# andrewcharlesjones/spatial-alignment

Hardware: AMD Instinct MI355X
Metric: training steps/sec (ELBO fwd+bwd), 2-view N=10k M=200, 1/2/4/8 GPU (higher is better)
Workload: dtype f32 (fp64 warp layer, covariance whitening and M x M factorisations)

## Files before the change

### include/gpsa_hip.h

```cpp
#ifndef GPSA_HIP_H
#define GPSA_HIP_H

#ifdef __cplusplus
extern "C" {
#endif

enum {
  GPSA_F32 = 0,
  GPSA_F64 = 1,
  GPSA_F32_X64 = 2,
  GPSA_F32_OUT64 = 3,
  GPSA_F32_ACC64 = 4
};
enum { GPSA_K_RBF = 0, GPSA_K_MATERN12 = 1, GPSA_K_MATERN32 = 2 };
enum { GPSA_EINVAL = -1, GPSA_EWORKSPACE = -2, GPSA_EUNSUPPORTED = -3 };

int gpsa_version(void);
const char* gpsa_build_arch(void);
const char* gpsa_source_hash(void);

int gpsa_kmat(int dtype, int in_dtype, int kind, const void* Z, int M, const void* X, long long C,
              int D, const void* ls_u, const void* var_u, double jitter, void* K, void* stream);

long long gpsa_kmat_bwd_workspace(int dtype, int M, long long C, int D);
// ... 119 lines not shown
                    double* out, void* workspace, long long workspace_bytes, void* stream);
int gpsa_loglik_bwd(const float* F, const float* Y, const float* noise_u, const double* gout, int S,
                    long long N, int P, float* dF, float* dnoise_u, void* workspace,
                    long long workspace_bytes, void* stream);

int gpsa_bdot(int dtype, const void* A, long long strideA, const void* B, long long strideB,
              long long n, int batch, void* out, void* workspace, long long workspace_bytes,
              void* stream);
int gpsa_add_diag(int dtype, void* A, int M, int batch, double s, void* stream);

int gpsa_mvn_kl_fwd(const double* Kinv, const double* logdetK, const double* Omega,
                    long long omega_stride, const double* logdetO, long long logdet_stride,
                    const double* Dm, const double* KD, int M, int L, double* kl, void* stream);
int gpsa_mvn_kl_bwd(const double* Kuu, const double* Kinv, const double* Omega, long long omega_stride,
                    const double* Oinv, long long oinv_stride, const double* Dm, const double* KD,
                    const double* g, int M, int L, double* dOmega, double* dDm, double* Sp,
                    void* stream);

int gpsa_mvn_kl_grouped_fwd(const double* mats, const double* inv, const double* logdet,
                            const int* om_idx, const int* pr_idx, const double* D, int M, int T,
                            double* kl, double* KD, void* stream);
int gpsa_mvn_kl_grouped_bwd(const double* mats, const double* inv, const int* om_idx,
                            const int* pr_list, const int* grp_off, const int* order, const double* D,
                            const double* KD, const double* g, int M, int T, int P, double* dOmega,
                            double* dD, double* S, void* stream);

int gpsa_elbo_fwd(const double* ll, int n_ll, const double* kl, int n_kl, double kl_scale, float* loss,
                  void* stream);
int gpsa_elbo_bwd(const float* gloss, int n_ll, int n_kl, double kl_scale, double* dll, double* dkl,
                  void* stream);

long long gpsa_kmeans_workspace(long long N, int D, int K);
int gpsa_kmeans_assign(const float* X, long long N, int D, const float* centres, int K, int* assign,
                       float* d2, void* stream);
int gpsa_kmeans_update(const float* X, const int* assign, long long N, int D, int K, float* centres,
                       int* counts, void* workspace, long long workspace_bytes, void* stream);


int gpsa_kmat_batched(int kind, const float* Z, long long strideZ, int M, const float* X, long long strideX,
                      long long C, int D, const float* ls_u, const float* var_u, int stride_par,
                      const long long* n_live, int batch, double jitter, double* K, long long strideK,
                      void* stream);
long long gpsa_kmat_bwd_batched_workspace(int M, long long C, int D, int batch);
int gpsa_kmat_bwd_batched(int kind, const float* Z, long long strideZ, int M, const float* X, long long strideX,
                          long long C, int D, const float* ls_u, const float* var_u, int stride_par,
                          const long long* n_live, int batch, const double* Kbar, long long strideK, int same,
                          double* dZ, long long stride_dZ, double* dparams, void* workspace,
                          long long workspace_bytes, void* stream);
int gpsa_kmat_bwd_x64(int kind, const float* Z, int M, const double* X, long long C, int D, const float* ls_u,
                      const float* var_u, const float* Kbar, double* dZ, double* dX, double* dparams,
                      void* workspace, long long workspace_bytes, void* stream);
int gpsa_kmat_bwd_x64_f64(int kind, const float* Z, int M, const double* X, long long C, int D, const float* ls_u,
                          const float* var_u, const double* Kbar, double* dZ, double* dX, double* dparams,
                          void* workspace, long long workspace_bytes, void* stream);
int gpsa_kmat_bwd_x64_f64_axpy(int kind, const float* Z, int M, const double* X, long long C, int D, const float* ls_u,
                               const float* var_u, const double* Kbar, const double* X2, const float* d, double s,
                               double* dZ, double* dX, double* dparams, void* workspace, long long workspace_bytes,
                               void* stream);
long long gpsa_exact_dkuu_workspace(int M, long long C);
int gpsa_exact_dkuu_f64(const double* G, const double* A, const float* d, int M, long long C, double* dK,
                        void* workspace, long long workspace_bytes, void* stream);
long long gpsa_longk_f64_workspace(int M, long long K, int nprob);
int gpsa_longk_f64(int nprob, const double* const* G, const double* const* B, const void* const* d, int d_dtype,
                   int M, long long K, long long ld, int sym, const double* alpha, const double* beta,
                   double* const* out, void* workspace, long long workspace_bytes, void* stream);
int gpsa_kmat_bwd_x64_axpy(int kind, const float* Z, int M, const double* X, long long C, int D, const float* ls_u,
                           const float* var_u, const float* Kbar, const float* X2, const float* d, double s,
                           double* dZ, double* dX, double* dparams, void* workspace, long long workspace_bytes,
                           void* stream);
int gpsa_whiten_f64_dual(const double* Kinv, const double* Kuf, int M, long long C, double* alpha64, float* alpha32,
                         double* q, void* workspace, long long workspace_bytes, void* stream);

int gpsa_whiten_gen_f64_dual(const double* Kinv, int kind, const float* Z, const double* X64, int D, const float* ls_u,
                             const float* var_u, int M, long long C, double* alpha64, float* alpha32, double* q,
                             void* workspace, long long workspace_bytes, void* stream);
int gpsa_whiten_axpy_f32(const double* Kinv, const float* X, int M, long long C, const float* X2, const float* d,
                         double s, float* out, void* workspace, long long workspace_bytes, void* stream);
int gpsa_whiten_batched_f64(const double* Kinv, long long strideKinv, const double* Kuf, int M, long long C,
                            long long strideX, double* alpha, double* q, int batch, void* workspace,
                            long long workspace_bytes, void* stream);
int gpsa_quadform_fwd_keep_batched_f64(const double* alpha, const double* Omega, int M, long long C, int L,
                                       double* v, double* W, const double* dcT, double* meanT, int batch,
                                       void* stream);
int gpsa_quadform_bwd_alpha_kept_batched_f64(const double* W, const double* g, int M, long long C, int L,
                                             const double* dcT, const double* dmeanT, double* dalpha,
                                             int batch, void* stream);
int gpsa_col_axpy_batched_f64(const double* Y, const double* X, const double* d, double s, int M, long long C,
                              double* out, int batch, void* stream);
long long gpsa_gram_batched_workspace(int M, long long C, int L, int batch);
int gpsa_gram_batched_f64(const double* alpha, const double* g, int M, long long C, int L, double* dOmega,
                          int batch, void* workspace, long long workspace_bytes, void* stream);
int gpsa_mvn_kl_grouped_bwd_acc(const double* mats, const double* inv, const int* om_idx,
                                const int* pr_list, const int* grp_off, const int* order, const double* D,
                                const double* KD, const double* g, int M, int T, int P, double* dOmega,
                                double* dD, double* S, int accumulate, void* stream);

#define GPSA_MAX_MODS 4

typedef struct gpsa_step_desc {
  int n_views, n_dims, n_mods, n_samples;
  int m_x, m_g;
  int kind_warp, kind_data;
  int n_latent[GPSA_MAX_MODS];
  int n_out[GPSA_MAX_MODS];
  int has_lmc[GPSA_MAX_MODS];
  long long n_rows[GPSA_MAX_MODS];
  int s_test;
  long long n_test[GPSA_MAX_MODS];
  int want_kl;
  const int* view_fixed;
  const long long* view_rows;
  long long keep_budget_bytes;
  int exact_inducing_grad;
  int kl_own_lo, kl_own_hi;
  int contraction;
} gpsa_step_desc;

typedef struct gpsa_step_params {
  const float* Xtilde;
  const float* delta_G;
  const float* Omega_sqt_G;
  const float* warp_ls;
  const float* warp_var;
  const float* slopes;
  const float* intercepts;
  const float* Gtilde;
  const float* data_ls;
  const float* data_var;
  const float* Omega_sqt_F[GPSA_MAX_MODS];
  const float* delta_F[GPSA_MAX_MODS];
  const float* W[GPSA_MAX_MODS];
} gpsa_step_params;

typedef struct gpsa_step_param_grads {
  float *Xtilde, *delta_G, *Omega_sqt_G, *warp_ls, *warp_var, *Gtilde, *data_ls, *data_var;
  float* Omega_sqt_F[GPSA_MAX_MODS];
  float* delta_F[GPSA_MAX_MODS];
  float* W[GPSA_MAX_MODS];
} gpsa_step_param_grads;

typedef struct gpsa_step_io {
  const float* X[GPSA_MAX_MODS];
  const float* eps_G;
  const float* eps_F[GPSA_MAX_MODS];
  const float* G_test[GPSA_MAX_MODS];
  const float* eps_F_test[GPSA_MAX_MODS];
  float* G_means[GPSA_MAX_MODS];
  float* G_samples[GPSA_MAX_MODS];
  float* F_latent[GPSA_MAX_MODS];
  float* F_obs[GPSA_MAX_MODS];
  float* F_latent_test[GPSA_MAX_MODS];
  float* F_obs_test[GPSA_MAX_MODS];
  float* mu_z;
  double* kl;
  int* flag;
  int keep_products;
  int reuse_mm;
  int fuse_elbo;
  const float* Y[GPSA_MAX_MODS];
  const float* noise_u[GPSA_MAX_MODS];
  double* ll_part[GPSA_MAX_MODS];
  float* F_fused_T[GPSA_MAX_MODS];
  double* bwd_acc;
  int bwd_acc_mode;
  void* f_event;
  const float* loss_src;
// ... 88 lines not shown
```

### spatial_alignment_amd/_lib.py

```python
import ctypes as C
import os

_HERE = os.path.dirname(os.path.abspath(__file__))
LIB_PATH = os.path.join(_HERE, "libgpsa_hip.so")

_vp, _i, _ll, _d = C.c_void_p, C.c_int, C.c_longlong, C.c_double

SIGNATURES = {
    "gpsa_version": (_i, []),
    "gpsa_build_arch": (C.c_char_p, []),
    "gpsa_source_hash": (C.c_char_p, []),
    "gpsa_kmat": (_i, [_i, _i, _i, _vp, _i, _vp, _ll, _i, _vp, _vp, _d, _vp, _vp]),
    "gpsa_kmat_bwd_workspace": (_ll, [_i, _i, _ll, _i]),
    "gpsa_kmat_bwd": (_i, [_i, _i, _i, _vp, _i, _vp, _ll, _i, _vp, _vp, _vp, _i, _vp, _vp, _vp, _vp, _ll, _vp]),
    "gpsa_gemm_workspace": (_ll, [_i, _i, _i, _i, _i]),
    "gpsa_gemm": (_i, [_i, _i, _i, _i, _i, _ll, _d, _vp, _ll, _ll, _vp, _ll, _ll, _d, _vp, _ll, _ll,
                       _i, _i, _vp, _ll, _vp]),
    "gpsa_omega_fwd": (_i, [_vp, _i, _i, _d, _vp, _vp]),
    "gpsa_omega_bwd": (_i, [_vp, _vp, _i, _i, _i, _vp, _vp]),
    "gpsa_omega_fwd2": (_i, [_vp, _i, _vp, _vp, _i, _vp, _i, _d, _vp]),
    "gpsa_omega_bwd2": (_i, [_vp, _vp, _vp, _i, _vp, _vp, _vp, _i, _i, _i, _vp]),
    "gpsa_chol_f64": (_i, [_vp, _i, _i, _vp, _vp, _vp]),
    "gpsa_tri_inv_f64": (_i, [_vp, _vp, _i, _i, _vp]),
    "gpsa_chol_inv_f64": (_i, [_vp, _vp, _i, _i, _vp, _vp, _vp]),
    "gpsa_experiment_split_bf16_product": (_i, [_vp, _vp, _i, _ll, _i, _i, _vp, _vp]),
    "gpsa_experiment_split_bf16_rate": (_i, [_i, _i, _vp, _vp]),
    "gpsa_chol_inv_sel_f64": (_i, [_vp, _vp, _i, _i, _i, _i, _i, _vp, _vp, _vp]),
    "gpsa_chol_inv_blocked_workspace": (_ll, [_i, _i]),
    "gpsa_chol_inv_blocked_f64": (_i, [_vp, _vp, _i, _i, _vp, _vp, _vp, _ll, _vp]),
    "gpsa_quadform_workspace": (_ll, [_i, _i, _ll, _i]),
    "gpsa_quadform_fwd": (_i, [_i, _i, _vp, _vp, _i, _ll, _i, _vp, _vp, _ll, _vp]),
    "gpsa_quadform_bwd_alpha": (_i, [_i, _i, _vp, _vp, _vp, _i, _ll, _i, _vp, _vp, _ll, _vp]),
    "gpsa_quadform_fwd_keep": (_i, [_i, _vp, _vp, _i, _ll, _i, _vp, _vp, _vp, _vp, _vp]),
    "gpsa_quadform_bwd_alpha_kept": (_i, [_i, _vp, _vp, _i, _ll, _i, _vp, _vp, _vp, _vp]),
    "gpsa_quadform_bwd_omega": (_i, [_i, _i, _vp, _vp, _i, _ll, _i, _vp, _vp, _ll, _vp]),
    "gpsa_quadform_bwd_omega_takes_delta": (_i, [_i, _ll]),
    "gpsa_quadform_bwd_omega_delta_f32": (_i, [_i, _vp, _vp, _vp, _i, _ll, _i, _vp, _vp, _d, _vp, _ll, _vp]),
    "gpsa_quadform_bwd_omega_x3_workspace": (_ll, [_i, _ll, _i]),
    "gpsa_quadform_bwd_omega_x3": (_i, [_i, _i, _vp, _vp, _i, _ll, _i, _vp, _vp, _ll, _vp]),
    "gpsa_quadform_bwd_omega_delta_x3": (_i, [_i, _vp, _vp, _vp, _i, _ll, _i, _vp, _vp, _d, _vp, _ll, _vp]),
    "gpsa_whiten_workspace": (_ll, [_i]),
    "gpsa_whiten_f64": (_i, [_vp, _i, _vp, _i, _ll, _i, _vp, _vp, _vp, _ll, _vp]),
    "gpsa_panel_mm": (_i, [_i, _i, _i, _vp, _vp, _i, _ll, _vp, _vp, _vp, _ll, _vp]),
    "gpsa_col_axpy": (_i, [_i, _vp, _vp, _vp, _d, _i, _ll, _vp, _vp]),
    "gpsa_data_sample_fwd": (_i, [_vp, _vp, _vp, _vp, _vp, _ll, _i, _vp, _vp, _vp]),
    "gpsa_data_sample_bwd": (_i, [_vp, _vp, _vp, _vp, _ll, _i, _vp, _vp, _vp, _i, _vp, _vp, _ll, _vp]),
    "gpsa_warp_sample_fwd": (_i, [_vp, _vp, _vp, _vp, _vp, _vp, _vp, _vp, _ll, _i, _i, _vp, _vp, _vp, _vp, _vp]),
    "gpsa_warp_sample_bwd": (_i, [_vp, _vp, _vp, _vp, _vp, _vp, _ll, _i, _i, _vp, _vp, _vp, _vp, _vp, _vp, _vp,
                                  _ll, _vp]),
    "gpsa_mean_resid_fwd": (_i, [_vp, _vp, _vp, _vp, _i, _i, _d, _vp, _vp, _vp]),
    "gpsa_mean_resid_bwd": (_i, [_vp, _vp, _vp, _i, _i, _d, _vp, _vp, _vp, _vp, _vp]),
    "gpsa_loglik_fwd": (_i, [_vp, _vp, _vp, _i, _ll, _i, _vp, _vp, _ll, _vp]),
    "gpsa_loglik_bwd": (_i, [_vp, _vp, _vp, _vp, _i, _ll, _i, _vp, _vp, _vp, _ll, _vp]),
    "gpsa_bdot": (_i, [_i, _vp, _ll, _vp, _ll, _ll, _i, _vp, _vp, _ll, _vp]),
    "gpsa_add_diag": (_i, [_i, _vp, _i, _i, _d, _vp]),
    "gpsa_mvn_kl_fwd": (_i, [_vp, _vp, _vp, _ll, _vp, _ll, _vp, _vp, _i, _i, _vp, _vp]),
    "gpsa_mvn_kl_bwd": (_i, [_vp, _vp, _vp, _ll, _vp, _ll, _vp, _vp, _vp, _i, _i, _vp, _vp, _vp, _vp]),
    "gpsa_mvn_kl_grouped_fwd": (_i, [_vp, _vp, _vp, _vp, _vp, _vp, _i, _i, _vp, _vp, _vp]),
    "gpsa_mvn_kl_grouped_bwd": (_i, [_vp, _vp, _vp, _vp, _vp, _vp, _vp, _vp, _vp, _i, _i, _i, _vp, _vp, _vp,
                                     _vp]),
    "gpsa_elbo_fwd": (_i, [_vp, _i, _vp, _i, _d, _vp, _vp]),
    "gpsa_elbo_bwd": (_i, [_vp, _i, _i, _d, _vp, _vp, _vp]),
    "gpsa_kmeans_workspace": (_ll, [_ll, _i, _i]),
    "gpsa_kmeans_assign": (_i, [_vp, _ll, _i, _vp, _i, _vp, _vp, _vp]),
    "gpsa_kmeans_update": (_i, [_vp, _vp, _ll, _i, _i, _vp, _vp, _vp, _ll, _vp]),
}

MAX_MODS = 4


class StepDesc(C.Structure):
    _fields_ = [
        ("n_views", _i), ("n_dims", _i), ("n_mods", _i), ("n_samples", _i),
        ("m_x", _i), ("m_g", _i), ("kind_warp", _i), ("kind_data", _i),
        ("n_latent", _i * MAX_MODS), ("n_out", _i * MAX_MODS), ("has_lmc", _i * MAX_MODS),
        ("n_rows", _ll * MAX_MODS), ("s_test", _i), ("n_test", _ll * MAX_MODS), ("want_kl", _i),
        ("view_fixed", C.POINTER(_i)), ("view_rows", C.POINTER(_ll)), ("keep_budget_bytes", _ll),
        ("exact_inducing_grad", _i), ("kl_own_lo", _i), ("kl_own_hi", _i), ("contraction", _i),
    ]


class StepParams(C.Structure):
    _fields_ = [
        ("Xtilde", _vp), ("delta_G", _vp), ("Omega_sqt_G", _vp), ("warp_ls", _vp), ("warp_var", _vp),
        ("slopes", _vp), ("intercepts", _vp), ("Gtilde", _vp), ("data_ls", _vp), ("data_var", _vp),
        ("Omega_sqt_F", _vp * MAX_MODS), ("delta_F", _vp * MAX_MODS), ("W", _vp * MAX_MODS),
    ]


class StepParamGrads(C.Structure):
    _fields_ = [
        ("Xtilde", _vp), ("delta_G", _vp), ("Omega_sqt_G", _vp), ("warp_ls", _vp), ("warp_var", _vp),
        ("Gtilde", _vp), ("data_ls", _vp), ("data_var", _vp),
        ("Omega_sqt_F", _vp * MAX_MODS), ("delta_F", _vp * MAX_MODS), ("W", _vp * MAX_MODS),
    ]


class StepIO(C.Structure):
    _fields_ = [
        ("X", _vp * MAX_MODS), ("eps_G", _vp), ("eps_F", _vp * MAX_MODS), ("G_test", _vp * MAX_MODS),
        ("eps_F_test", _vp * MAX_MODS), ("G_means", _vp * MAX_MODS), ("G_samples", _vp * MAX_MODS),
        ("F_latent", _vp * MAX_MODS), ("F_obs", _vp * MAX_MODS), ("F_latent_test", _vp * MAX_MODS),
        ("F_obs_test", _vp * MAX_MODS), ("mu_z", _vp), ("kl", _vp), ("flag", _vp), ("keep_products", _i),
        ("reuse_mm", _i), ("fuse_elbo", _i), ("Y", _vp * MAX_MODS), ("noise_u", _vp * MAX_MODS),
        ("ll_part", _vp * MAX_MODS), ("F_fused_T", _vp * MAX_MODS), ("bwd_acc", _vp), ("bwd_acc_mode", _i),
        ("f_event", _vp), ("loss_src", _vp), ("loss_dst", _vp),
    ]


class StepOutGrads(C.Structure):
    _fields_ = [
        ("dG_means", _vp * MAX_MODS), ("dG_samples", _vp * MAX_MODS), ("dF_latent", _vp * MAX_MODS),
        ("dF_obs", _vp * MAX_MODS), ("dF_latent_test", _vp * MAX_MODS), ("dF_obs_test", _vp * MAX_MODS),
        ("dkl", _vp), ("gloss", _vp),
    ]


_pp = C.POINTER(_vp)

SIGNATURES.update({
    "gpsa_kmat_batched": (_i, [_i, _vp, _ll, _i, _vp, _ll, _ll, _i, _vp, _vp, _i, C.POINTER(_ll), _i, _d, _vp, _ll, _vp]),
    "gpsa_kmat_bwd_batched_workspace": (_ll, [_i, _ll, _i, _i]),
    "gpsa_kmat_bwd_batched": (_i, [_i, _vp, _ll, _i, _vp, _ll, _ll, _i, _vp, _vp, _i, C.POINTER(_ll), _i, _vp, _ll, _i,
                                   _vp, _ll, _vp, _vp, _ll, _vp]),
# ... 148 lines not shown
```

### spatial_alignment_amd/csrc/step.hip

```cpp
#include <stdint.h>
#include <stdio.h>
#include <stdlib.h>
#include <string.h>

#include <new>
#include <vector>

#include "internal.hpp"

namespace gpsa {

constexpr int MAXMODS = GPSA_MAX_MODS;
constexpr int KM_MAXB_STEP = 16;

struct Arena {
  char* base = nullptr;
  long long off = 0, high = 0;
  long long limit = -1;
  bool dry = false;
  bool overflow = false;
  template <typename T>
  T* get(long long n) {
    off = (off + 255) & ~255LL;
    T* p = dry ? nullptr : reinterpret_cast<T*>(base + off);
// ... 1039 lines not shown
      if (G.M > 256)
        GPSA_RUN(gpsa_chol_inv_blocked_f64(c.mats(G, o0), LinvO[g], G.M, n_own, logdet + o0, info + o0, wsO[g],
                                           wsOb[g], (void*)sst));
      else
        GPSA_RUN(gpsa_chol_inv_f64(c.mats(G, o0), LinvO[g], G.M, n_own, logdet + o0, info + o0, (void*)sst));
      GPSA_RUN((gemm_launch_tri<double>(1, 0, G.M, G.M, G.M, 1.0, LinvO[g], G.M, mm, LinvO[g], G.M, mm, 0.0,
                                        c.inv(G, o0), G.M, mm, n_own, 1, nullptr, 0, sst, GEMM_TRI_LTL)));
    }
  }
  if (fork) {
    GPSA_CK((int)hipEventRecord(P.sev[1], c.st));
    GPSA_CK((int)hipStreamWaitEvent(P.side, P.sev[1], 0));
  }
  if (kl)
    for (int g = 0; g < P.ng; ++g) {
      Group& G = P.grp[g];
      if (G.n_omega > 0)
        GPSA_RUN(mvn_kl_grouped_fwd_copy(c.mats(G, 0), c.inv(G, 0), c.sv<double>(G.o_logdet), G.om_idx, G.pr_idx,
                                         c.sv<double>(G.o_D), G.M, G.n_omega, c.io.kl + G.kl_off,
                                         c.sv<double>(G.o_KD), c.sv<double>(P.o_klcache) + G.kl_off, klpart[g], klcnt[g],
                                         sst));
    }
  if (fork) GPSA_CK((int)hipEventRecord(P.sev[2], P.side));
  return 0;
}

static ModPtrs mod_ptrs(Ctx& c, const gpsa_step_out_grads* og, const double* const* dG64) {
  ModPtrs p;
  memset(&p, 0, sizeof(p));
  for (int m = 0; m < c.P.nm; ++m) {
    p.X[m] = c.io.X[m];
    p.Gm[m] = c.io.G_means[m];
    p.Gs[m] = c.io.G_samples[m];
    p.G64[m] = c.sv<double>(c.P.o_G64[m]);
    p.N[m] = c.P.d.n_rows[m];
    if (og != nullptr) {
      p.dGm[m] = og->dG_means[m];
      p.dGs[m] = og->dG_samples[m];
    }
    if (dG64 != nullptr) p.dG64[m] = dG64[m];
  }
  return p;
}

static int project_views(Ctx& c, const double* Kinv, const double* Kuf, int M, long long Cs, double* alpha,
                         double* q, int cnt, int b0, bool packed) {
  const bool dry = c.dry;
  const long long wsb1 = gpsa_whiten_workspace(M);
  if (wsb1 > 0) {
    void* ws = c.sv<char>(c.P.o_apk_w) + wsb1 * b0;
    GPSA_RUN(gpsa_whiten_batched_f64(packed ? nullptr : Kinv, (long long)M * M, Kuf, M, Cs, (long long)M * Cs, alpha, q,
                                     cnt, ws, wsb1 * cnt, c.stv()));
    return 0;
  }
  GPSA_CK(gemm64(c, 0, 0, M, (int)Cs, M, 1.0, Kinv, M, (long long)M * M, Kuf, Cs, (long long)M * Cs, 0.0, alpha,
                 Cs, (long long)M * Cs, cnt, 1));
  if (q != nullptr && !dry) {
    dim3 grid((unsigned)cdiv(Cs, 256), (unsigned)cnt);
    coldot2_kernel<<<grid, 256, 0, c.st>>>(Kuf, alpha, M, Cs, q);
    GPSA_LAUNCH_CHECK();
  }
  return 0;
}

static int warp_stage_fwd(Ctx& c) {
  Plan& P = c.P;
  const bool dry = c.dry;
  const int V = P.V, D = P.D, Mx = P.Mx, nf = P.nf;
  const long long Cs = P.Cs;
  Group& GW = P.gw();
  (void)V;
  const long long mk = c.sc.mark();
  double* meanT = nullptr;
  double* vq = nullptr;
  double* q = nullptr;
  if (nf > 0 && Cs > 0) {
    float* Xv = c.sv<float>(P.o_Xv);
    double* alpha = c.sv<double>(P.o_alpha_w);
    double* Wk = c.sv<double>(P.o_Wk);
    meanT = c.sc.get<double>((long long)nf * D * Cs);
    vq = c.sc.get<double>((long long)nf * D * Cs);
    q = c.sc.get<double>((long long)nf * Cs);
    double* Kuf = c.sc.get<double>((long long)nf * Mx * Cs);
    if (!dry) {
      dim3 grid((unsigned)cdiv(Cs, 256), (unsigned)nf);
      warp_gather_kernel<<<grid, 256, 0, c.st>>>(P.tab, P.d_free, mod_ptrs(c, nullptr, nullptr), Xv);
      GPSA_LAUNCH_CHECK();
    }
    for (const Run& r : P.runs) {
      long long nlive[KM_MAXB_STEP];
      for (int i = 0; i < r.cnt; ++i) nlive[i] = P.nview[r.v0 + i];
      GPSA_RUN(gpsa_kmat_batched(P.d.kind_warp, c.prm.Xtilde + (long long)r.v0 * Mx * D, (long long)Mx * D, Mx,
                                 Xv + (long long)r.b0 * Cs * D, Cs * D, Cs, D, c.prm.warp_ls + r.v0,
                                 c.prm.warp_var + r.v0, 1, nlive, r.cnt, 0.0, Kuf + (long long)r.b0 * Mx * Cs,
                                 (long long)Mx * Cs, c.stv()));
      GPSA_CK(project_views(c, c.inv(GW, P.pos_Kw(r.b0)), Kuf + (long long)r.b0 * Mx * Cs, Mx, Cs,
                            alpha + (long long)r.b0 * Mx * Cs, q + (long long)r.b0 * Cs, r.cnt, r.b0, false));
      GPSA_RUN(gpsa_quadform_fwd_keep_batched_f64(
          alpha + (long long)r.b0 * Mx * Cs, c.mats(GW, P.pos_OmG(r.v0 * D)), Mx, Cs, D,
          vq + (long long)r.b0 * D * Cs, Wk + (long long)r.b0 * D * Mx * Cs,
          c.sv<double>(P.o_resid) + (long long)r.v0 * Mx * D, meanT + (long long)r.b0 * D * Cs, r.cnt, c.stv()));
    }
  }
  int* bad = c.sv<int>(P.o_bad);
  long long boff = 0;
  for (int m = 0; m < P.nm; ++m) {
    const long long N = P.d.n_rows[m];
    if (N == 0) continue;
    const long long nb = cdiv(N, 256);
    if (!dry) {
      warp_sample_views_fwd_kernel<<<(unsigned)nb, 256, 0, c.st>>>(
          P.tab, m, c.io.X[m], meanT, vq, q, c.prm.warp_var, c.prm.slopes, c.prm.intercepts, c.io.eps_G, N,
          c.io.G_means[m], c.io.G_samples[m], c.sv<double>(P.o_G64[m]), bad + boff);
      GPSA_LAUNCH_CHECK();
    }
    boff += nb;
  }
  c.sc.release(mk);
  if (P.d.want_kl && P.side != nullptr && !dry) GPSA_CK((int)hipStreamWaitEvent(c.st, P.sev[2], 0));
  if (c.io.flag != nullptr && !dry) {
    Group& G0 = P.grp[0];
    const int n0 = P.d.want_kl ? G0.nb() : G0.n_prior;
    flag_reduce_kernel<<<1, 256, 0, c.st>>>(c.sv<int>(G0.o_info), n0, bad, P.nbad, c.io.flag);
    GPSA_LAUNCH_CHECK();
    if (P.ng == 2) {
      Group& G1 = P.grp[1];
      const int n1 = P.d.want_kl ? G1.nb() : G1.n_prior;
      flag_reduce_kernel<<<1, 256, 0, c.st>>>(c.sv<int>(G1.o_info), n1, c.io.flag, 1, c.io.flag);
      GPSA_LAUNCH_CHECK();
    }
  }
  return 0;
}

static int data_pass_fwd(Ctx& c, const Pass& ps) {
  Plan& P = c.P;
  const bool dry = c.dry;
  const int m = ps.m, Mg = P.Mg, D = P.D, L = P.d.n_latent[m], Pm = P.d.n_out[m];
  const long long C = ps.C;
  Group& GD = P.gd();
  const double* Kinv = c.inv(GD, P.pos_KF());
  const double* Om = c.mats(GD, P.pos_OmF(m, 0));
  float* alpha = c.sv<float>(ps.o_alpha);
  float* Sigma = c.sv<float>(ps.o_sigma);
  const float* eps = ps.test ? c.io.eps_F_test[m] : c.io.eps_F[m];
  float* F = ps.test ? c.io.F_latent_test[m] : c.io.F_latent[m];
  float* Fo = ps.test ? c.io.F_obs_test[m] : c.io.F_obs[m];
  const long long mk = c.sc.mark();
  double* q = c.sc.get<double>(C);
  {
    const long long mk2 = c.sc.mark();
    double* Kuf = c.sc.get<double>((long long)Mg * C);
    const long long wsb = gpsa_whiten_workspace(Mg);
    const bool exact = ps.o_alpha64 >= 0;
    bool fused = false;
    if (!ps.test && exact && wsb > 0 && !dry) {
      if (c.sc.overflow) return GPSA_EWORKSPACE;
      const int rc = gpsa_whiten_gen_f64_dual(c.apk_d ? nullptr : Kinv, P.d.kind_data, c.prm.Gtilde,
                                              c.sv<double>(P.o_G64[m]), D, c.prm.data_ls, c.prm.data_var, Mg, C,
                                              c.sv<double>(ps.o_alpha64), alpha, q, c.sv<char>(P.o_apk_d), wsb, c.stv());
      if (rc == 0) fused = true, c.apk_d = true;
      else if (rc != GPSA_EUNSUPPORTED) return rc;
    }
    if (!fused) {
      if (ps.test)
        GPSA_RUN(gpsa_kmat(GPSA_F64, GPSA_F32, P.d.kind_data, c.prm.Gtilde, Mg, c.io.G_test[m], C, D, c.prm.data_ls,
                           c.prm.data_var, 0.0, Kuf, c.stv()));
      else
        GPSA_RUN(gpsa_kmat(GPSA_F64, GPSA_F32_X64, P.d.kind_data, c.prm.Gtilde, Mg, c.sv<double>(P.o_G64[m]), C, D,
                           c.prm.data_ls, c.prm.data_var, 0.0, Kuf, c.stv()));
      if (wsb > 0 && !exact) {
        void* ws = c.sv<char>(P.o_apk_d);
        GPSA_RUN(gpsa_whiten_f64(c.apk_d ? nullptr : Kinv, GPSA_F64, Kuf, Mg, C, GPSA_F32, alpha, q, ws, wsb,
                                 c.stv()));
// ... 1110 lines not shown
```

Measured before the change: 150.6.

## Fuse warp-layer kernel eval, whitening and quadform into one persistent MFMA kernel

Adds a persistent fp64 MFMA kernel that computes Kuf on the fly per 16-column group, multiplies it by the packed Kinv and Omega matrices, and emits alpha, W, q, v and meanT in a single pass. This replaces the separate kmat, whitening projection and quadform launches for the warp layer. It removes the materialised Kuf round trip through memory and the extra launches, using a pre-packed register-friendly layout for the M x M matrices. In exchange it adds a pack kernel, heavy register pressure at one wave per SIMD, and padding of M to 7 or 13 tiles. It also changes the launch to a grid capped at the CU count.

```diff
diff --git a/include/gpsa_hip.h b/include/gpsa_hip.h
--- a/include/gpsa_hip.h
+++ b/include/gpsa_hip.h
@@ -225,6 +225,13 @@
 int gpsa_quadform_fwd_keep_batched_f64(const double* alpha, const double* Omega, int M, long long C, int L,
                                        double* v, double* W, const double* dcT, double* meanT, int batch,
                                        void* stream);
+int gpsa_warp_fwd_fused_ok(int kind, int M, int D, int batch);
+int gpsa_warp_fused_grid(long long C, int batch);
+long long gpsa_warp_fused_deal(long long C, int batch, int nwg, int wg, long long* u0, long long* u1);
+int gpsa_warp_fwd_fused_f64(int kind, const double* Kinv, const double* Omega, const float* Z, const float* X,
+                            const float* ls_u, const float* var_u, const long long* n_live, const double* dcT, int M,
+                            long long C, int D, int batch, double* alpha, double* W, double* q, double* v,
+                            double* meanT, void* ws_kinv, void* ws_omega, void* stream);
 int gpsa_quadform_bwd_alpha_kept_batched_f64(const double* W, const double* g, int M, long long C, int L,
                                              const double* dcT, const double* dmeanT, double* dalpha,
                                              int batch, void* stream);
diff --git a/spatial_alignment_amd/_lib.py b/spatial_alignment_amd/_lib.py
--- a/spatial_alignment_amd/_lib.py
+++ b/spatial_alignment_amd/_lib.py
@@ -40,6 +40,11 @@
     "gpsa_quadform_bwd_omega_x3": (_i, [_i, _i, _vp, _vp, _i, _ll, _i, _vp, _vp, _ll, _vp]),
     "gpsa_quadform_bwd_omega_delta_x3": (_i, [_i, _vp, _vp, _vp, _i, _ll, _i, _vp, _vp, _d, _vp, _ll, _vp]),
     "gpsa_whiten_workspace": (_ll, [_i]),
+    "gpsa_warp_fwd_fused_ok": (_i, [_i, _i, _i, _i]),
+    "gpsa_warp_fused_grid": (_i, [_ll, _i]),
+    "gpsa_warp_fused_deal": (_ll, [_ll, _i, _i, _i, _vp, _vp]),
+    "gpsa_warp_fwd_fused_f64": (_i, [_i, _vp, _vp, _vp, _vp, _vp, _vp, _vp, _vp, _i, _ll, _i, _i, _vp, _vp, _vp, _vp,
+                                     _vp, _vp, _vp, _vp]),
     "gpsa_whiten_f64": (_i, [_vp, _i, _vp, _i, _ll, _i, _vp, _vp, _vp, _ll, _vp]),
     "gpsa_panel_mm": (_i, [_i, _i, _i, _vp, _vp, _i, _ll, _vp, _vp, _vp, _ll, _vp]),
     "gpsa_col_axpy": (_i, [_i, _vp, _vp, _vp, _d, _i, _ll, _vp, _vp]),
diff --git a/spatial_alignment_amd/csrc/step.hip b/spatial_alignment_amd/csrc/step.hip
--- a/spatial_alignment_amd/csrc/step.hip
+++ b/spatial_alignment_amd/csrc/step.hip
@@ -1145,6 +1145,8 @@
     vq = c.sc.get<double>((long long)nf * D * Cs);
     q = c.sc.get<double>((long long)nf * Cs);
     double* Kuf = c.sc.get<double>((long long)nf * Mx * Cs);
+    const long long wsb_w = gpsa_whiten_workspace(Mx);
+    char* Opk = c.sc.get<char>(wsb_w * nf * D);
     if (!dry) {
       dim3 grid((unsigned)cdiv(Cs, 256), (unsigned)nf);
       warp_gather_kernel<<<grid, 256, 0, c.st>>>(P.tab, P.d_free, mod_ptrs(c, nullptr, nullptr), Xv);
@@ -1153,6 +1155,17 @@
     for (const Run& r : P.runs) {
       long long nlive[KM_MAXB_STEP];
       for (int i = 0; i < r.cnt; ++i) nlive[i] = P.nview[r.v0 + i];
+      static const bool fused_off = [] { const char* e = getenv("GPSA_WARP_FUSED"); return e && e[0] == '0'; }();
+      if (!fused_off && wsb_w > 0 && gpsa_warp_fwd_fused_ok(P.d.kind_warp, Mx, D, r.cnt)) {
+        GPSA_RUN(gpsa_warp_fwd_fused_f64(
+            P.d.kind_warp, c.inv(GW, P.pos_Kw(r.b0)), c.mats(GW, P.pos_OmG(r.v0 * D)),
+            c.prm.Xtilde + (long long)r.v0 * Mx * D, Xv + (long long)r.b0 * Cs * D, c.prm.warp_ls + r.v0,
+            c.prm.warp_var + r.v0, nlive, c.sv<double>(P.o_resid) + (long long)r.v0 * Mx * D, Mx, Cs, D, r.cnt,
+            alpha + (long long)r.b0 * Mx * Cs, Wk + (long long)r.b0 * D * Mx * Cs, q + (long long)r.b0 * Cs,
+            vq + (long long)r.b0 * D * Cs, meanT + (long long)r.b0 * D * Cs, c.sv<char>(P.o_apk_w) + wsb_w * r.b0,
+            Opk + wsb_w * (long long)r.b0 * D, c.stv()));
+        continue;
+      }
       GPSA_RUN(gpsa_kmat_batched(P.d.kind_warp, c.prm.Xtilde + (long long)r.v0 * Mx * D, (long long)Mx * D, Mx,
                                  Xv + (long long)r.b0 * Cs * D, Cs * D, Cs, D, c.prm.warp_ls + r.v0,
                                  c.prm.warp_var + r.v0, 1, nlive, r.cnt, 0.0, Kuf + (long long)r.b0 * Mx * Cs,
diff --git a/spatial_alignment_amd/csrc/warp_fused.hip b/spatial_alignment_amd/csrc/warp_fused.hip
--- /dev/null
+++ b/spatial_alignment_amd/csrc/warp_fused.hip
@@ -0,0 +1,284 @@
+#include "internal.hpp"
+#include "kmat_cov.hpp"
+
+#include <stdlib.h>
+
+namespace gpsa {
+
+typedef double wf_f64x4 __attribute__((ext_vector_type(4)));
+
+constexpr int WF_GROUP = 16;
+constexpr int WF_MAXB = 16;
+
+__host__ __device__ inline void wf_deal(long long U, int nwg, int wg, long long& u0, long long& u1) {
+  u0 = (long long)wg * U / nwg;
+  u1 = (long long)(wg + 1) * U / nwg;
+}
+
+struct WarpFwdArgs {
+  const double* Apk;
+  const double* Opk;
+  const float* Z;
+  const float* X;
+  const float *ls, *var;
+  const double* dcT;
+  double *alpha, *W, *q, *v, *meanT;
+  long long n[WF_MAXB];
+  long long C, G, U;
+  int M;
+};
+
+__global__ void __launch_bounds__(256) warp_pack_kernel(const double* __restrict__ Kinv, const double* __restrict__ Omega,
+                                                        int M, int MB, int D, double* __restrict__ Apk,
+                                                        double* __restrict__ Opk) {
+  const long long idx = blockIdx.x * 256LL + threadIdx.x;
+  const long long tot = (long long)MB * 4 * MB * 64;
+  if (idx >= tot) return;
+  const int b = blockIdx.y / (1 + D), p = blockIdx.y % (1 + D);
+  const double* src = p == 0 ? Kinv + (long long)b * M * M : Omega + ((long long)b * D + p - 1) * M * M;
+  double* dst = p == 0 ? Apk + b * tot : Opk + ((long long)b * D + p - 1) * tot;
+  const int lane = (int)(idx & 63);
+  long long t = idx >> 6;
+  const int rt = (int)(t % MB);
+  t /= MB;
+  const int row = rt * 16 + (lane & 15), k = (int)t * 4 + (lane >> 4);
+  dst[idx] = (row < M && k < M) ? src[(long long)row * M + k] : 0.0;
+}
+
+template <int MB, int KIND, int ND>
+__global__ void __launch_bounds__(256, 1) warp_fwd_fused_kernel(WarpFwdArgs a) {
+  constexpr long long PBD = (long long)MB * 4 * MB * 64;
+  constexpr int NST = (1 + ND) * MB;
+  __shared__ double red[4][MB][4][64];
+  __shared__ double Zs[MB * 16][ND];
+  __shared__ double sm[4][1 + 2 * ND][16];
+
+  const int tid = threadIdx.x, lane = tid & 63;
+  const int w = __builtin_amdgcn_readfirstlane(tid >> 6);
+  const int j = lane & 15, kq = lane >> 4;
+  long long u0, u1;
+  wf_deal(a.U, (int)gridDim.x, (int)blockIdx.x, u0, u1);
+  if (u0 >= u1) return;
+  const long long C = a.C;
+  const int M = a.M;
+
+  const long long lane_off = (long long)w * MB * MB * 64 + lane;
+  auto mat_of = [&](int b, int p) -> const double* {
+    return (p == 0 ? a.Apk + (long long)b * PBD : a.Opk + ((long long)b * ND + (p - 1)) * PBD) + lane_off;
+  };
+
+  int bz = -1;
+  double ell = 1.0, inv_ell = 1.0, var = 1.0;
+  double ac[MB], an[MB];
+#pragma unroll
+  for (int t = 0; t < MB; ++t) an[t] = 0.0;
+  {
+    const int b = (int)(u0 / a.G);
+    const double* m0 = mat_of(b, 0);
+#pragma unroll
+    for (int t = 0; t < MB; ++t) ac[t] = m0[(long long)t * MB * 64];
+  }
+  for (long long u = u0; u < u1; ++u) {
+    const int b = (int)(u / a.G);
+    const long long c = (u % a.G) * WF_GROUP + j;
+    const bool okc = c < C, livec = c < a.n[b];
+    if (b != bz) {
+      __syncthreads();
+      for (int i = tid; i < MB * 16 * ND; i += 256) {
+        const int r = i / ND, d = i % ND;
+        Zs[r][d] = (double)a.Z[((long long)b * M + (r < M ? r : M - 1)) * ND + d];
+      }
+      ell = exp((double)a.ls[b]);
+      inv_ell = 1.0 / ell;
+      var = exp((double)a.var[b]);
+      bz = b;
+      __syncthreads();
+    }
+    double rhs[MB], kb[MB];
+    {
+      double x[MAXD];
+#pragma unroll
+      for (int d = 0; d < MAXD; ++d) x[d] = d < ND ? (double)a.X[((long long)b * C + (okc ? c : 0)) * ND + d] : 0.0;
+#pragma unroll
+      for (int t = 0; t < MB; ++t) {
+        double k, cd, pl;
+        cov_eval<double, KIND>(Zs[4 * (w * MB + t) + kq], x, ND, ell, inv_ell, var, k, cd, pl);
+        kb[t] = livec ? k : 0.0;
+        rhs[t] = kb[t];
+      }
+    }
+    double al[MB];
+    double s_q = 0.0, s_v[ND], s_m[ND];
+#pragma unroll
+    for (int d = 0; d < ND; ++d) s_v[d] = s_m[d] = 0.0;
+
+#pragma unroll
+    for (int st = 0; st < NST; ++st) {
+      const int p = st / MB, rt = st % MB;
+      if (st + 1 < NST) {
+        const double* mn = mat_of(b, (st + 1) / MB) + ((st + 1) % MB) * 64;
+#pragma unroll
+        for (int t = 0; t < MB; ++t) an[t] = mn[(long long)t * MB * 64];
+      } else if (u + 1 < u1) {
+        const double* mn = mat_of((int)((u + 1) / a.G), 0);
+#pragma unroll
+        for (int t = 0; t < MB; ++t) an[t] = mn[(long long)t * MB * 64];
+      }
+      __builtin_amdgcn_sched_barrier(0);
+      wf_f64x4 acc0 = (wf_f64x4){0.0, 0.0, 0.0, 0.0}, acc1 = (wf_f64x4){0.0, 0.0, 0.0, 0.0};
+#pragma unroll
+      for (int t = 0; t < MB; ++t) {
+        if (t & 1) acc1 = __builtin_amdgcn_mfma_f64_16x16x4f64(ac[t], rhs[t], acc1, 0, 0, 0);
+        else acc0 = __builtin_amdgcn_mfma_f64_16x16x4f64(ac[t], rhs[t], acc0, 0, 0, 0);
+      }
+      __builtin_amdgcn_sched_barrier(0);
+#pragma unroll
+      for (int r = 0; r < 4; ++r) red[w][rt][r][lane] = acc0[r] + acc1[r];
+#pragma unroll
+      for (int t = 0; t < MB; ++t) ac[t] = an[t];
+
+      if (rt == MB - 1) {
+        __syncthreads();
+        double y[MB];
+#pragma unroll
+        for (int t = 0; t < MB; ++t) {
+          const int s = w * MB + t;
+          const double* rp = &red[0][s >> 2][s & 3][lane];
+          y[t] = (rp[0] + rp[MB * 256]) + (rp[2 * MB * 256] + rp[3 * MB * 256]);
+        }
+        double* out = p == 0 ? a.alpha + (long long)b * M * C : a.W + ((long long)b * ND + (p - 1)) * M * C;
+#pragma unroll
+        for (int t = 0; t < MB; ++t) {
+          const int row = 4 * (w * MB + t) + kq;
+          if (okc && row < M) out[(long long)row * C + c] = y[t];
+        }
+        if (p == 0) {
+#pragma unroll
+          for (int t = 0; t < MB; ++t) {
+            const int row = 4 * (w * MB + t) + kq;
+            al[t] = y[t];
+            rhs[t] = y[t];
+            s_q += y[t] * kb[t];
+            const double* dc = a.dcT + ((long long)b * M + (row < M ? row : M - 1)) * ND;
+#pragma unroll
+            for (int d = 0; d < ND; ++d) s_m[d] += y[t] * dc[d];
+          }
+        } else {
+#pragma unroll
+          for (int t = 0; t < MB; ++t) s_v[p - 1] += al[t] * y[t];
+        }
+        __syncthreads();
+      }
+    }
+    {
+      double z[1 + 2 * ND];
+      z[0] = s_q;
+#pragma unroll
+      for (int d = 0; d < ND; ++d) z[1 + d] = s_v[d], z[1 + ND + d] = s_m[d];
+#pragma unroll
+      for (int i = 0; i < 1 + 2 * ND; ++i) {
+        z[i] += __shfl_xor(z[i], 16, 64);
+        z[i] += __shfl_xor(z[i], 32, 64);
+        if (kq == 0) sm[w][i][j] = z[i];
+      }
+      __syncthreads();
+      if (w == 0 && okc) {
+        for (int i = kq; i < 1 + 2 * ND; i += 4) {
+          const double r = (sm[0][i][j] + sm[1][i][j]) + (sm[2][i][j] + sm[3][i][j]);
+          if (i == 0) a.q[(long long)b * C + c] = r;
+          else if (i <= ND) a.v[((long long)b * ND + (i - 1)) * C + c] = r;
+          else a.meanT[((long long)b * ND + (i - 1 - ND)) * C + c] = r;
+        }
+      }
+    }
+  }
+}
+
+static inline int wf_mb_for(int M) {
+  const int mb = (M + 15) / 16;
+  if (mb <= 7 && mb > 4) return 7;
+  if (mb <= 13 && mb > 7) return 13;
+  return 0;
+}
+
+}
+
+extern "C" {
+
+int gpsa_warp_fwd_fused_ok(int kind, int M, int D, int batch) {
+  using namespace gpsa;
+  if (wf_mb_for(M) == 0 || D < 1 || D > 2 || batch < 1 || batch > WF_MAXB) return 0;
+  return kind == GPSA_K_RBF || kind == GPSA_K_MATERN12 || kind == GPSA_K_MATERN32;
+}
+
+long long gpsa_warp_fused_deal(long long C, int batch, int nwg, int wg, long long* u0, long long* u1) {
+  using namespace gpsa;
+  if (C < 1 || batch < 1 || nwg < 1 || wg < 0 || wg >= nwg) return GPSA_EINVAL;
+  const long long U = cdiv(C, WF_GROUP) * batch;
+  long long x0, x1;
+  wf_deal(U, nwg, wg, x0, x1);
+  if (u0) *u0 = x0;
+  if (u1) *u1 = x1;
+  return U;
+}
+
+int gpsa_warp_fused_grid(long long C, int batch) {
+  using namespace gpsa;
+  if (C < 1 || batch < 1) return GPSA_EINVAL;
+  const long long U = cdiv(C, WF_GROUP) * batch;
+  return (int)(U < num_cus() ? U : num_cus());
+}
+
+int gpsa_warp_fwd_fused_f64(int kind, const double* Kinv, const double* Omega, const float* Z, const float* X,
+                            const float* ls_u, const float* var_u, const long long* n_live, const double* dcT, int M,
+                            long long C, int D, int batch, double* alpha, double* W, double* q, double* v,
+                            double* meanT, void* ws_kinv, void* ws_omega, void* stream) {
+  using namespace gpsa;
+  if (M < 1 || C < 1 || !Kinv || !Omega || !Z || !X || !ls_u || !var_u || !dcT || !alpha || !W || !q || !v || !meanT ||
+      !ws_kinv || !ws_omega)
+    return GPSA_EINVAL;
+  if (!gpsa_warp_fwd_fused_ok(kind, M, D, batch)) return GPSA_EUNSUPPORTED;
+  const int MB = wf_mb_for(M);
+  hipStream_t st = as_stream(stream);
+  const long long tot = (long long)MB * 4 * MB * 64;
+  warp_pack_kernel<<<dim3((unsigned)cdiv(tot, 256), (unsigned)(batch * (1 + D))), 256, 0, st>>>(
+      Kinv, Omega, M, MB, D, (double*)ws_kinv, (double*)ws_omega);
+  GPSA_LAUNCH_CHECK();
+  WarpFwdArgs a;
+  a.Apk = (const double*)ws_kinv;
+  a.Opk = (const double*)ws_omega;
+  a.Z = Z;
+  a.X = X;
+  a.ls = ls_u;
+  a.var = var_u;
+  a.dcT = dcT;
+  a.alpha = alpha;
+  a.W = W;
+  a.q = q;
+  a.v = v;
+  a.meanT = meanT;
+  for (int i = 0; i < WF_MAXB; ++i) a.n[i] = i < batch ? (n_live ? n_live[i] : C) : 0;
+  a.C = C;
+  a.G = cdiv(C, WF_GROUP);
+  a.U = a.G * batch;
+  a.M = M;
+  const unsigned grid = (unsigned)gpsa_warp_fused_grid(C, batch);
+#define GPSA_WF(MB_, K_, D_)                                              \
+  warp_fwd_fused_kernel<MB_, K_, D_><<<grid, 256, 0, st>>>(a);
+#define GPSA_WF_K(MB_, D_)                                                \
+  switch (kind) {                                                         \
+    case GPSA_K_RBF: GPSA_WF(MB_, GPSA_K_RBF, D_) break;                  \
+    case GPSA_K_MATERN12: GPSA_WF(MB_, GPSA_K_MATERN12, D_) break;        \
+    default: GPSA_WF(MB_, GPSA_K_MATERN32, D_) break;                     \
+  }
+  if (MB == 13 && D == 2) GPSA_WF_K(13, 2)
+  else if (MB == 13) GPSA_WF_K(13, 1)
+  else if (D == 2) GPSA_WF_K(7, 2)
+  else GPSA_WF_K(7, 1)
+#undef GPSA_WF_K
+#undef GPSA_WF
+  GPSA_LAUNCH_CHECK();
+  return 0;
+}
+
+}
```

New measurement: 151.3 (median of 6 runs). Within noise of the previous version (+0.4%).
